# AnyLoc/Revisit-Anything

Measured on AMD Instinct MI355X. Metric: query_images_per_sec, higher is better.
Workload: dtype f32

## Files before the change

### revisit-anything_amd/csrc/api.hip

```cpp
#include <stdarg.h>
#include <stdlib.h>
#include <string.h>

#include <cmath>
#include <mutex>
#include <utility>

#include <initializer_list>

#include "ctx.h"

int segvlad_ctx::fail(int code, const char* fmt, ...) {
  va_list ap;
  va_start(ap, fmt);
  vsnprintf(err, sizeof(err), fmt, ap);
  va_end(ap);
  return code;
}

bool sv_is_device_ptr(const void* p) {
  hipPointerAttribute_t a;
  memset(&a, 0, sizeof(a));
  hipError_t e = hipPointerGetAttributes(&a, p);
  if (e != hipSuccess) {
// ... 199 lines not shown
  *out = c;
  return SEGVLAD_OK;
}

int segvlad_set_option(segvlad_ctx* ctx, const char* key, const char* value) {
  if (!ctx) return SEGVLAD_ERR_ARG;
  if (!key || !value) return ctx->fail(SEGVLAD_ERR_ARG, "set_option: null key/value");
  SvOptions& o = ctx->opt;
  auto as_int = [&](int* dst) -> int {
    char* end = nullptr;
    const long v = strtol(value, &end, 10);
    if (end == value || *end) return ctx->fail(SEGVLAD_ERR_ARG, "set_option(%s): '%s' is not an integer", key, value);
    *dst = (int)v;
    return SEGVLAD_OK;
  };
  if (!strcmp(key, "knn_filter")) {
    if (!strcmp(value, "auto")) o.knn_filter = 0;
    else if (!strcmp(value, "f16")) o.knn_filter = 1;
    else if (!strcmp(value, "bf16x3")) o.knn_filter = 2;
    else if (!strcmp(value, "fp32")) o.knn_filter = 3;
    else return ctx->fail(SEGVLAD_ERR_ARG, "set_option(knn_filter): want auto|f16|bf16x3|fp32, got '%s'", value);
    return SEGVLAD_OK;
  }
  if (!strcmp(key, "pca_arith")) {
    if (!strcmp(value, "auto") || !strcmp(value, "f16x3")) o.pca_fp32 = 0;
    else if (!strcmp(value, "fp32")) o.pca_fp32 = 1;
    else return ctx->fail(SEGVLAD_ERR_ARG, "set_option(pca_arith): want auto|f16x3|fp32, got '%s'", value);
    return SEGVLAD_OK;
  }
  if (!strcmp(key, "pca_path")) {
    if (!strcmp(value, "auto")) o.pca_path = 0;
    else if (!strcmp(value, "planes")) o.pca_path = 1;
    else if (!strcmp(value, "project")) o.pca_path = 2;
    else return ctx->fail(SEGVLAD_ERR_ARG, "set_option(pca_path): want auto|planes|project, got '%s'", value);
    return SEGVLAD_OK;
  }
  if (!strcmp(key, "vlad_assign")) {
    if (!strcmp(value, "hard")) {
      o.vlad_soft_temp = 0.f, o.vlad_soft_pooled = 0;
      return SEGVLAD_OK;
    }
    const int pooled = !strncmp(value, "soft_pooled:", 12);
    if (pooled || !strncmp(value, "soft:", 5)) {
      const char* t = value + (pooled ? 12 : 5);
      bool decimal = *t != 0 && (*t == '.' || (*t >= '0' && *t <= '9'));
      for (const char* c = t; *c && decimal; ++c) decimal = strchr("0123456789.eE+-", *c) != nullptr;
      char* end = nullptr;
      const float temp = decimal ? strtof(t, &end) : 0.f;
      if (decimal && end != t && *end == 0 && std::isfinite(temp) && temp > 0.f) {
        o.vlad_soft_temp = temp, o.vlad_soft_pooled = pooled;
        return SEGVLAD_OK;
      }
    }
    return ctx->fail(SEGVLAD_ERR_ARG, "set_option(vlad_assign): want hard|soft:<T>|soft_pooled:<T> with a finite decimal T > 0, got '%s'", value);
  }
  auto as_dev = [&](int* dst, std::initializer_list<int> product_values, std::initializer_list<int> probe_values = {}) -> int {
    int v = *dst;
    SV_TRY(as_int(&v));
    bool ok = false;
    for (int a : product_values) ok = ok || a == v;
#ifdef SEGVLAD_ABLATIONS
    for (int a : probe_values) ok = ok || a == v;
#else
    (void)probe_values;
#endif
    if (!ok)
      return ctx->fail(SEGVLAD_ERR_ARG, "set_option(%s=%d): a development switch -- this library holds the default kernels only "
                       "(SEGVLAD_BUILD_ABLATIONS=1 builds lib/libsegvlad_hip_abl.so with the probes of csrc/segvlad_dev.h)", key, v);
    *dst = v;
    return SEGVLAD_OK;
  };
  if (!strcmp(key, "f16_cfg")) return as_dev(&o.f16_cfg, {-1, 250, 300, 62, 63}, {93, 94, 95});
  if (!strcmp(key, "f16_gm")) return as_int(&o.f16_gm);
  if (!strcmp(key, "f16_walk")) return as_int(&o.f16_walk);
  if (!strcmp(key, "f16_deep_cfg")) return as_dev(&o.f16_deep_cfg, {-1, 4, 5});
  if (!strcmp(key, "f16_buf")) return as_dev(&o.f16_buf, {-1, 0});
  if (!strcmp(key, "tnk_gram")) return as_int(&o.tnk_gram);
  if (!strcmp(key, "tnk_fork")) return as_int(&o.tnk_fork);
  if (!strcmp(key, "x3_tile")) return as_int(&o.x3_tile);
  if (!strcmp(key, "x3_gm")) return as_int(&o.x3_gm);
  if (!strcmp(key, "search_stats")) return as_int(&o.search_stats);
  if (!strcmp(key, "knn_heuristic")) return as_int(&o.knn_heuristic);
  if (!strcmp(key, "assign_narrow")) return as_int(&o.assign_narrow);
  if (!strcmp(key, "agg_kpb")) return as_int(&o.agg_kpb);
  if (!strcmp(key, "pj_nw")) return as_int(&o.pj_nw);
  if (!strcmp(key, "pj_f16")) return as_int(&o.pj_f16);
  if (!strcmp(key, "cover_rows")) return as_int(&o.cover_rows);
  if (!strcmp(key, "pj_planes")) return as_int(&o.pj_planes);
  if (!strcmp(key, "small_plan")) return as_int(&o.small_plan);
  if (!strcmp(key, "small_tail")) return as_int(&o.small_tail);
  if (!strcmp(key, "small_head")) return as_int(&o.small_head);
  if (!strcmp(key, "batch_l0_f16")) return as_int(&o.batch_l0_f16);
  if (!strcmp(key, "level_carry")) return as_int(&o.level_carry);
  if (!strcmp(key, "f16_persist_wgs")) return as_int(&o.f16_persist_wgs);
  if (!strcmp(key, "debug_small_tail")) return as_int(&o.debug_small_tail);
  if (!strcmp(key, "refine_group")) return as_int(&o.refine_group);
  if (!strcmp(key, "query_group")) return as_int(&o.query_group);
  if (!strcmp(key, "group_fetch")) return as_int(&o.group_fetch);
  if (!strcmp(key, "debug_search")) return as_int(&o.debug_search);
  if (!strcmp(key, "debug_fail_search")) return as_int(&o.debug_fail_search);
  if (!strcmp(key, "guard_undersize")) {
    if (!ctx->guard) return ctx->fail(SEGVLAD_ERR_STATE, "set_option(guard_undersize): the context was not created under SEGVLAD_GUARD=1");
    const char* colon = strchr(value, ':');
    bool found = false;
    ctx->for_each_buf([&](DevBuf& b) {
      if (!colon) b.shrink = 0;
      else if (strlen(b.tag) == (size_t)(colon - value) && !strncmp(b.tag, value, (size_t)(colon - value))) {
        b.shrink = atoi(colon + 1);
        found = true;
      }
    });
    if (colon && !found) return ctx->fail(SEGVLAD_ERR_ARG, "set_option(guard_undersize): no buffer named like '%s'", value);
    return SEGVLAD_OK;
  }
  return ctx->fail(SEGVLAD_ERR_ARG, "set_option: unknown key '%s'", key);
}

int segvlad_destroy(segvlad_ctx* ctx) {
  if (!ctx) return SEGVLAD_OK;
  (void)hipSetDevice(ctx->device);
  (void)hipStreamSynchronize(ctx->stream);
  sv_comm_release(ctx);
  if (ctx->side) {
    (void)hipStreamSynchronize(ctx->side);
    (void)hipStreamDestroy(ctx->side);
    (void)hipEventDestroy(ctx->ev_fork);
    (void)hipEventDestroy(ctx->ev_join);
  }
  if (ctx->h_pin) {
    (void)hipHostFree(ctx->h_pin);
    (void)hipEventDestroy(ctx->ev_scalars);
  }
  if (ctx->h_desc) (void)hipHostFree(ctx->h_desc);
  if (ctx->ev_desc) (void)hipEventDestroy(ctx->ev_desc);
  ctx->for_each_buf([](DevBuf& b) { b.release(); });
  for (auto& kv : ctx->timers)
    for (hipEvent_t e : kv.second.ev)
      if (e) (void)hipEventDestroy(e);
  delete ctx;
  return SEGVLAD_OK;
}

const char* segvlad_last_error(const segvlad_ctx* ctx) { return ctx ? ctx->err : "null context"; }

int segvlad_set_stream(segvlad_ctx* ctx, void* hip_stream) {
  if (!ctx) return SEGVLAD_ERR_ARG;
  ctx->stream = reinterpret_cast<hipStream_t>(hip_stream);
  return SEGVLAD_OK;
}

int segvlad_synchronize(segvlad_ctx* ctx) {
  CHECK_CTX();
  SV_HIP(hipStreamSynchronize(ctx->stream));
  return sv_guard_check(ctx);
}

int segvlad_set_profiling(segvlad_ctx* ctx, int on) {
  if (!ctx) return SEGVLAD_ERR_ARG;
  ctx->profiling = on != 0;
  return SEGVLAD_OK;
}

int segvlad_profile_reset(segvlad_ctx* ctx) {
  if (!ctx) return SEGVLAD_ERR_ARG;
  for (auto& kv : ctx->timers) {
    kv.second.used = 0;
// ... 290 lines not shown
```

### revisit-anything_amd/csrc/ctx.h

```cpp
#pragma once
#include <hip/hip_runtime.h>
#include <math.h>
#include <stdint.h>
#include <stdio.h>
#include <string.h>

#include <map>
#include <string>
#include <vector>

#include "../../include/segvlad.h"

#define SV_HIP(expr)                                                                              \
  do {                                                                                            \
    hipError_t _e = (expr);                                                                       \
    if (_e != hipSuccess) {                                                                       \
      return ctx->fail(SEGVLAD_ERR_HIP, "%s failed: %s (%s:%d)", #expr, hipGetErrorString(_e),    \
                       __FILE__, __LINE__);                                                       \
    }                                                                                             \
  } while (0)

#define SV_TRY(expr)          \
  do {                        \
    int _r = (expr);          \
// ... 11 lines not shown
}
#endif

#if defined(__HIPCC__)
__host__ __device__
#endif
inline int sv_x3_swz(int64_t row) { return (int)((0 - (row >> 2)) & 3); }
#if defined(__HIPCC__)
__host__ __device__
#endif
inline size_t sv_x3_off(int64_t row, int64_t k, int64_t Kd) {
  return ((size_t)(row >> 7) * (size_t)(Kd >> 5) + (size_t)(k >> 5)) * 4096 + (size_t)(row & 127) * 32 +
         (size_t)((((k & 31) >> 3) ^ sv_x3_swz(row)) << 3) + (size_t)(k & 7);
}
inline int64_t sv_x3_rows(int64_t n) { return (n + 255) & ~255ll; }
inline float sv_fp16_scale(float bound) {
  int e;
  frexpf(bound, &e);
  return ldexpf(1.f, 14 - e);
}

constexpr size_t SV_GUARD_BYTES = 1024;
constexpr uint32_t SV_GUARD_WORD = 0xA5C3F00Du;
struct DevBuf {
  void* p = nullptr;
  size_t cap = 0;
  const char* tag = "";
  bool guard = false;
  bool fixed = false;
  void* raw = nullptr;
  size_t req = 0;
  int shrink = 0;
  hipError_t reserve(size_t bytes) {
    if (guard) return reserve_guarded(bytes);
    if (bytes <= cap) return hipSuccess;
    if (p) {
      hipError_t e = hipFree(p);
      if (e != hipSuccess) return e;
      p = nullptr;
      cap = 0;
    }
    size_t want = bytes + bytes / 8 + 256;
    hipError_t e = hipMalloc(&p, want);
    if (e != hipSuccess) return e;
    cap = want;
    return hipSuccess;
  }
  hipError_t reserve_guarded(size_t bytes);
  size_t fence_off() const { return fixed ? cap : ((req > (size_t)shrink ? req - (size_t)shrink : 0) + 3) & ~(size_t)3; }
  void release() {
    if (raw) (void)hipFree(raw);
    else if (p) (void)hipFree(p);
    raw = nullptr;
    p = nullptr;
    cap = 0;
    req = 0;
  }
  template <class T>
  T* as() { return reinterpret_cast<T*>(p); }
};

struct StageTimer {
  std::vector<hipEvent_t> ev;
  int used = 0;
  int launches = 0;
};

struct SvOptions {
  int knn_filter = 0;
  int pca_fp32 = 0;
  int f16_cfg = -1;
  int f16_gm = -1;
  int f16_walk = -1;
  int f16_persist_wgs = 32;
  int f16_deep_cfg = -1;
  int f16_buf = -1;
  int tnk_gram = 1;
  int tnk_fork = 1;
  int x3_tile = 0;
  int x3_gm = -1;
  int search_stats = 0;
  int knn_heuristic = 1;
  int assign_narrow = 0;
  int agg_kpb = 4;
  int debug_fail_search = 0;
  int debug_search = 0;
  int debug_small_tail = 0;
  int batch_l0_f16 = 1;
  int level_carry = 1;
  int small_head = 1;
  int small_tail = 1;
  int small_plan = 1;
  int pj_f16 = 1;
  int pj_nw = 8;
  int refine_group = 1;
  int query_group = 0;
  int pca_path = 0;
  int cover_rows = 1;
  int pj_planes = 1;
  float vlad_soft_temp = 0.f;
  int vlad_soft_pooled = 0;
  int group_fetch = 0;
};

constexpr int SV_F16_KBLOCK = 1024;
inline int sv_f16_kblock(const SvOptions& o, int d) {
  if (o.f16_cfg == 300) return SV_F16_KBLOCK;
  return (o.f16_cfg < 0 && d >= 4096) ? SV_F16_KBLOCK : 0;
}
constexpr int SV_F16_KFLUSH = 64;
int sv_f16_eps_kblock(const SvOptions& o, int d);
inline bool sv_f16_bias_possible(const SvOptions& o, int64_t nq) { return nq > 128 && (o.f16_cfg < 0 || o.f16_cfg == 250 || o.f16_cfg == 300); }
enum class F16Kernel {
  None, BatchDefault, BatchComplement, BatchSmall, BatchUnbiased, BatchUnbiasedSmall, DeepFlush, DeepFlushComplement, DeepBlockedBuf, DeepBlocked,
  DeepBlockedBufComplement, DeepBlockedComplement, DeepUnbiased, OneImage64, OneImage128,
#ifdef SEGVLAD_ABLATIONS
  ProbePhases, ProbeNoEpilogue, ProbeNoEpilogueNoDma,
#endif
};
struct F16Choice {
  F16Kernel kernel;
  const char* why;
};
F16Choice sv_choose_f16_kernel(const SvOptions& o, bool bias_ok, int M, int64_t n_rows, int d, int b_stride, int skip);
inline float sv_f16_c_eps(int d, int kb, float bias_mult) {
  const float acc = kb > 0 ? (2.f * (float)kb + (float)((d + kb - 1) / kb) + 1.f) / 16777216.f : 2.f * (float)d / 16777216.f;
  return 2.5f * (1.f / 1024.f + 1.f / 4194304.f + bias_mult * acc);
}

struct SvSearchStats {
  int64_t levels = 0;
  int64_t filter = 0;
  int64_t n_fallback = 0;
  int64_t cand_max = 0;
  int64_t cand_sum = 0;
  int64_t refine_max = 0;
  int64_t refine_sum = 0;
  int64_t n_queries = 0;
  int64_t n_redo = 0;
  int64_t n_refine2 = 0;
  int64_t grp_groups = 0;
  int64_t grp_union_sum = 0;
  int64_t carry_rows = 0;
};

struct OpenDescribe {
  bool open = false;
  bool side_pending = false;
  int B = 0, S_tot = 0;
  StageTimer* timer = nullptr;
  int slot = 0;
};

struct segvlad_ctx {
  int device = 0;
  hipStream_t stream = nullptr;
  hipStream_t side = nullptr;
  hipEvent_t ev_fork = nullptr, ev_join = nullptr;
  uint32_t* h_pin = nullptr;
  hipEvent_t ev_scalars = nullptr;
  unsigned char* h_desc = nullptr;
  size_t h_desc_cap = 0;
  hipEvent_t ev_desc = nullptr;
  OpenDescribe desc;
  char err[512] = {0};
  bool profiling = false;
// ... 318 lines not shown
```

### revisit-anything_amd/csrc/vlad_kernels.hip

```cpp
#include <stdio.h>
#include <stdlib.h>

#include "ctx.h"
#include "incidence_dev.h"

typedef float f32x16 __attribute__((ext_vector_type(16)));

#define MFMA32(a, b, c) __builtin_amdgcn_mfma_f32_32x32x2f32((a), (b), (c), 0, 0, 0)

template <int CTRL>
__device__ __forceinline__ float dpp_f32(float x) {
  return __int_as_float(__builtin_amdgcn_update_dpp(0, __float_as_int(x), CTRL, 0xf, 0xf, true));
}

__device__ __forceinline__ int frag_row(int r, int kk) { return (r & 3) + 8 * (r >> 2) + 4 * kk; }

__global__ void vocab_norm_kernel(const float* __restrict__ C, int K, int D, float* __restrict__ inv) {
  const int k = blockIdx.x;
  float s = 0.f;
  for (int d = threadIdx.x; d < D; d += blockDim.x) {
    float v = C[(size_t)k * D + d];
    s = fmaf(v, v, s);
  }
  __shared__ float red[256];
// ... 394 lines not shown
      const float* bp = bt + ((size_t)((dbase >> 1) + st) * NT) * 64 + l;
#pragma unroll
      for (int n = 0; n < NT; ++n) {
        const float bv = bp[n * 64];
        if (ABL == 1) {
          acc[0][n][0] += x0 * bv;
          acc[1][n][0] += x1 * bv;
        } else {
          acc[0][n] = MFMA32(x0, bv, acc[0][n]);
          acc[1][n] = MFMA32(x1, bv, acc[1][n]);
        }
      }
      if (ABL != 2) {
        tile[(2 * i) * 65 + 2 * st + kk] = x0;
        tile[(2 * i + 1) * 65 + 2 * st + kk] = x1;
      }
    }
    __builtin_amdgcn_fence(__ATOMIC_RELEASE, "wavefront");
    __builtin_amdgcn_wave_barrier();
    __builtin_amdgcn_fence(__ATOMIC_ACQUIRE, "wavefront");
#pragma unroll 4
    for (int it = 0; it < 16; ++it) {
      const int idx = it * 64 + l;
      const int tok = idx >> 4, c4 = (idx & 15) << 2;
      if (ABL != 2 && ABL != 3 && t0 + tok < N && dbase + c4 < D) {
        const float* q = tile + tok * 65 + c4;
        float4 v = make_float4(q[0], q[1], q[2], q[3]);
        *reinterpret_cast<float4*>(Xt + ((size_t)b * N + t0 + tok) * D + dbase + c4) = v;
      }
    }
    __builtin_amdgcn_fence(__ATOMIC_RELEASE, "wavefront");
    __builtin_amdgcn_wave_barrier();
    __builtin_amdgcn_fence(__ATOMIC_ACQUIRE, "wavefront");
  }
  ss0 += __shfl_xor(ss0, 32);
  ss1 += __shfl_xor(ss1, 32);
  __syncthreads();
  constexpr int KP = NT * 32;
  float* sc = lds;
  float* ssum = lds + 64 * (KP + 1);
  if (kk == 0) {
    ssum[w * 64 + 2 * i] = ss0;
    ssum[w * 64 + 2 * i + 1] = ss1;
  }
  for (int rnd = 0; rnd < 4; ++rnd) {
    if (w == rnd) {
#pragma unroll
      for (int mt = 0; mt < 2; ++mt)
#pragma unroll
        for (int n = 0; n < NT; ++n)
#pragma unroll
          for (int r = 0; r < 16; ++r) {
            const int tok = 2 * frag_row(r, kk) + mt;
            float* p = &sc[tok * (KP + 1) + n * 32 + i];
            *p = (rnd == 0) ? acc[mt][n][r] : (*p + acc[mt][n][r]);
          }
    }
    __syncthreads();
  }
  if (tid < 64 && t0 + tid < N) {
    const float s2 = ((ssum[tid] + ssum[64 + tid]) + ssum[128 + tid]) + ssum[192 + tid];
    const float rn = 1.0f / fmaxf(sqrtf(s2), 1e-12f);
    float best = -INFINITY, second = -INFINITY;
    int bi = 0;
    for (int k = 0; k < K; ++k) {
      const float v = sc[tid * (KP + 1) + k];
      if (v > best) {
        second = best;
        best = v;
        bi = k;
      } else if (v > second) {
        second = v;
      }
    }
    const size_t o = (size_t)b * N + t0 + tid;
    labels[o] = (uint8_t)bi;
    rnorm[o] = rn;
    if (gap) gap[o] = (K > 1) ? (best - second) * rn : INFINITY;
  }
}

typedef float f32x4u __attribute__((ext_vector_type(4), aligned(4)));

template <int NT>
__device__ __forceinline__ void assign_wide_chunk(const float* __restrict__ tl, const float* __restrict__ bt, float* __restrict__ Xt,
                                                  int b, int N, int D, int t0, int tid, int w, int l, int i, int kk, int c,
                                                  f32x16 (&acc)[NT], float& ss) {
  constexpr int DC = 32, TS = 128;
  auto rot = [](int d) { return 8 * (d >> 2) + 32 * (d & 1); };
#pragma unroll 8
  for (int st = 0; st < DC / 2; ++st) {
    const float x = tl[(2 * st + kk) * TS + ((32 * w + i + rot(2 * st + kk)) & 127)];
    ss = fmaf(x, x, ss);
    const float* bp = bt + ((size_t)(c * (DC / 2) + st) * NT) * 64 + l;
#pragma unroll
    for (int n = 0; n < NT; ++n) acc[n] = MFMA32(x, bp[n * 64], acc[n]);
  }
#pragma unroll
  for (int it = 0; it < 4; ++it) {
    const int idx = it * 256 + tid;
    const int tok = idx >> 3, c4 = idx & 7;
    if (t0 + tok < N) {
      const float* q = tl + (4 * c4) * TS;
      const int t_a = (tok + 8 * c4) & 127, t_b = (tok + 8 * c4 + 32) & 127;
      const float4 o = make_float4(q[t_a], q[TS + t_b], q[2 * TS + t_a], q[3 * TS + t_b]);
      *reinterpret_cast<float4*>(Xt + ((size_t)b * N + t0 + tok) * D + c * DC + 4 * c4) = o;
    }
  }
}

template <int NT>
__global__ __launch_bounds__(256) void assign_wide_kernel(const float* __restrict__ T, int N, int D, int K,
                                                          const float* __restrict__ bt, float* __restrict__ Xt,
                                                          uint8_t* __restrict__ labels, float* __restrict__ rnorm,
                                                          float* __restrict__ gap, int B) {
  constexpr int DC = 32, TS = 128;
  auto rot = [](int d) { return 8 * (d >> 2) + 32 * (d & 1); };
  __shared__ __attribute__((aligned(16))) float tile[2 * DC * TS + 128];
  __shared__ float ssum[128];
  const int gx = (N + 127) / 128;
  const int per = (int)((gridDim.x + 7) / 8);
  const int logical = (int)(blockIdx.x & 7) * per + (int)(blockIdx.x >> 3);
  if (logical >= gx * B) return;
  const int b = logical / gx, t0 = (logical - b * gx) * 128;
  const int tid = threadIdx.x, w = tid >> 6, l = tid & 63, i = l & 31, kk = l >> 5;
  const float* Tb = T + (size_t)b * D * N;
  const int lr = tid >> 5, lq = tid & 31;
  const int tl0 = t0 + 4 * lq;
  const int nvalid = N - tl0;
  f32x16 acc[NT];
#pragma unroll
  for (int n = 0; n < NT; ++n)
#pragma unroll
    for (int r = 0; r < 16; ++r) acc[n][r] = 0.f;
  float ss = 0.f;
  const int nch = D / DC;
  float4 va[4], vb[4];
#define SV_LOAD_CHUNK(V, c)                                                           \
  _Pragma("unroll") for (int j = 0; j < 4; ++j) {                                     \
    const float* p = Tb + (size_t)((c) * DC + lr + 8 * j) * N + tl0;                  \
    if (nvalid >= 4) {                                                                \
      const f32x4u u = *reinterpret_cast<const f32x4u*>(p);                           \
      V[j] = make_float4(u[0], u[1], u[2], u[3]);                                     \
    } else {                                                                          \
      V[j] = make_float4(nvalid > 0 ? p[0] : 0.f, nvalid > 1 ? p[1] : 0.f, nvalid > 2 ? p[2] : 0.f, 0.f); \
    }                                                                                 \
  }
#define SV_PARK_CHUNK(V, buf)                                                         \
  _Pragma("unroll") for (int j = 0; j < 4; ++j) {                                     \
    const int d_ = lr + 8 * j;                                                        \
    float* q = tile + (buf) * (DC * TS) + d_ * TS + ((4 * lq + rot(d_)) & 127);       \
    *reinterpret_cast<float4*>(q) = V[j];                                             \
  }
  SV_LOAD_CHUNK(va, 0)
  SV_PARK_CHUNK(va, 0)
  if (1 < nch) { SV_LOAD_CHUNK(va, 1) }
  __syncthreads();
#define SV_ASSIGN_STEP(c, VNEXT, VFREE)                                               \
  {                                                                                   \
    if ((c) + 2 < nch) { SV_LOAD_CHUNK(VFREE, (c) + 2) }                              \
    assign_wide_chunk<NT>(tile + ((c) & 1) * (DC * TS), bt, Xt, b, N, D, t0, tid, w, l, i, kk, (c), acc, ss);  \
    if ((c) + 1 < nch) { SV_PARK_CHUNK(VNEXT, ((c) + 1) & 1) }                        \
    __syncthreads();                                                                  \
  }
  for (int c = 0; c < nch; c += 2) {
    SV_ASSIGN_STEP(c, va, vb)
    if (c + 1 < nch) SV_ASSIGN_STEP(c + 1, vb, va)
  }
#undef SV_ASSIGN_STEP
#undef SV_LOAD_CHUNK
#undef SV_PARK_CHUNK
  constexpr int KP = NT * 32;
  float* sc = tile;
  ss += __shfl_xor(ss, 32);
  if (kk == 0) ssum[32 * w + i] = ss;
#pragma unroll
  for (int n = 0; n < NT; ++n)
#pragma unroll
    for (int r = 0; r < 16; ++r) sc[(32 * w + frag_row(r, kk)) * (KP + 1) + n * 32 + i] = acc[n][r];
  __syncthreads();
  if (tid < 128 && t0 + tid < N) {
    const float rn = 1.0f / fmaxf(sqrtf(ssum[tid]), 1e-12f);
    float best = -INFINITY, second = -INFINITY;
    int bi = 0;
    for (int k = 0; k < K; ++k) {
      const float sv = sc[tid * (KP + 1) + k];
      if (sv > best) {
        second = best;
        best = sv;
        bi = k;
      } else if (sv > second) {
        second = sv;
      }
    }
    const size_t o = (size_t)b * N + t0 + tid;
    labels[o] = (uint8_t)bi;
    rnorm[o] = rn;
    if (gap) gap[o] = (K > 1) ? (best - second) * rn : INFINITY;
  }
}

int sv_launch_assign(segvlad_ctx* ctx, const float* tokens, int B, int N, float* xt, uint8_t* labels, float* rnorm,
                     float* gap) {
  const int NT = ctx->Kpad / 32;
  dim3 grid((N + 63) / 64, B), block(256);
  const float* bt = ctx->vocab_bt.as<float>();
  if (NT <= 2 && ctx->D % 32 == 0 && !ctx->opt.assign_narrow) {
    const unsigned tiles_total = (unsigned)((N + 127) / 128) * (unsigned)B;
    dim3 gridw((tiles_total + 7) / 8 * 8, 1);
    if (NT == 1)
      hipLaunchKernelGGL(assign_wide_kernel<1>, gridw, block, 0, ctx->stream, tokens, N, ctx->D, ctx->K, bt, xt, labels, rnorm, gap, B);
    else
      hipLaunchKernelGGL(assign_wide_kernel<2>, gridw, block, 0, ctx->stream, tokens, N, ctx->D, ctx->K, bt, xt, labels, rnorm, gap, B);
    SV_HIP(hipGetLastError());
    return SEGVLAD_OK;
  }
  switch (NT) {
    case 1:
      hipLaunchKernelGGL(assign_kernel<1>, grid, block, 0, ctx->stream, tokens, N, ctx->D, ctx->K, bt, xt, labels, rnorm, gap);
      break;
    case 2: {
#ifdef SEGVLAD_ABLATIONS
      const char* ab = getenv("SEGVLAD_ASSIGN_ABL");
      const int a = ab ? atoi(ab) : 0;
      if (a == 1) {
        hipLaunchKernelGGL((assign_kernel<2, 1>), grid, block, 0, ctx->stream, tokens, N, ctx->D, ctx->K, bt, xt, labels, rnorm, gap);
        break;
      } else if (a == 2) {
        hipLaunchKernelGGL((assign_kernel<2, 2>), grid, block, 0, ctx->stream, tokens, N, ctx->D, ctx->K, bt, xt, labels, rnorm, gap);
        break;
      } else if (a == 3) {
        hipLaunchKernelGGL((assign_kernel<2, 3>), grid, block, 0, ctx->stream, tokens, N, ctx->D, ctx->K, bt, xt, labels, rnorm, gap);
        break;
      }
#endif
      hipLaunchKernelGGL(assign_kernel<2>, grid, block, 0, ctx->stream, tokens, N, ctx->D, ctx->K, bt, xt, labels, rnorm, gap);
      break;
    }
    case 4:
      hipLaunchKernelGGL(assign_kernel<4>, grid, block, 0, ctx->stream, tokens, N, ctx->D, ctx->K, bt, xt, labels, rnorm, gap);
      break;
    default:
      return ctx->fail(SEGVLAD_ERR_LIMIT, "K=%d: supported cluster counts are 1..64 and 97..128 (Kpad in {32,64,128})", ctx->K);
  }
  SV_HIP(hipGetLastError());
  return SEGVLAD_OK;
}

__global__ __launch_bounds__(256) void prep_kernel(const uint8_t* __restrict__ labels, const uint64_t* __restrict__ inc,
                                                   const int32_t* __restrict__ seg_off,
                                                   const int64_t* __restrict__ adj_off, const uint8_t* __restrict__ adj,
                                                   int N, int K, int S_max, int SC, uint64_t* __restrict__ colmask,
                                                   float* __restrict__ gscale, int32_t* __restrict__ tok_order,
                                                   int32_t* __restrict__ lab_off, const float* __restrict__ rnorm,
                                                   float* __restrict__ rn_sorted, int stage, int ord_n,
                                                   int32_t* __restrict__ phys, int32_t* __restrict__ cov_cnt, int cover) {
  extern __shared__ __attribute__((aligned(16))) unsigned char smem[];
  const int b = blockIdx.x;
  const int nw = (N + 63) >> 6;
  const int s0 = seg_off[b], S = seg_off[b + 1] - s0;
  uint64_t* inc2 = reinterpret_cast<uint64_t*>(smem);
  uint64_t* lbits = inc2 + (size_t)S_max * nw;
  const int tid = threadIdx.x;
  if (adj && stage) {
    const int SW = (S_max + 63) >> 6;
    uint64_t* inc0 = reinterpret_cast<uint64_t*>(reinterpret_cast<int*>(lbits + (size_t)K * nw) + ord_n);
    uint64_t* nbr = inc0 + (size_t)S_max * nw;
    for (int idx = tid; idx < S * nw; idx += 256) inc0[idx] = inc[(size_t)s0 * nw + idx];
    for (int idx = tid; idx < S * SW; idx += 256) nbr[idx] = 0;
    __syncthreads();
    const uint8_t* a = adj + adj_off[b];
    for (int e = tid; e < S * S; e += 256)
      if (a[e]) {
        const int s = e / S, u = e - s * S;
        atomicOr(reinterpret_cast<unsigned long long*>(&nbr[s * SW + (u >> 6)]), 1ull << (u & 63));
      }
    __syncthreads();
    for (int idx = tid; idx < S * nw; idx += 256) {
      const int s = idx / nw, w = idx - s * nw;
      uint64_t v = 0;
      for (int uw = 0; uw < SW; ++uw) {
        uint64_t m = nbr[s * SW + uw];
        while (m) {
          const int u = (uw << 6) + __builtin_ctzll(m);
          m &= m - 1;
          v |= inc0[u * nw + w];
        }
      }
      inc2[idx] = v;
    }
  } else {
    for (int idx = tid; idx < S * nw; idx += 256) {
// ... 453 lines not shown
        if (single && dummy_row >= 0) {
          if (f >= TNK_QD && rem >= TNK_QD - 1) {
            if (sc == 0) asm volatile("s_waitcnt vmcnt(23)" ::: "memory");
            else asm volatile("s_waitcnt vmcnt(7)" ::: "memory");
          } else {
            tnk_wait_vm((rem < TNK_QD - 1 ? rem : TNK_QD - 1) + (sc == 0 ? 2 * (f < TNK_QD ? f : TNK_QD) : 0));
          }
        } else {
          asm volatile("s_waitcnt vmcnt(0)" ::: "memory");
        }
        if (single)
          lds_step_read(lds_addr(qbase + (f % TNK_QD) * 1024 + l * 16), lds_addr(rnl + j), lds_addr(mskl + j), x, rn, m);
        else
          x = lds_read_f32x4(lds_addr(qbase + (f % TNK_QD) * 1024 + l * 16));
        if (fi < total) issue();
        if (!dvalid) x = f32x4{0.f, 0.f, 0.f, 0.f};
        const float b0 = fmaf(x.x, rn, -c4.x), b1 = fmaf(x.y, rn, -c4.y);
        const float b2 = fmaf(x.z, rn, -c4.z), b3 = fmaf(x.w, rn, -c4.w);
        if (sc == 0) {
          typedef _Float16 h4 __attribute__((ext_vector_type(4)));
          const float fv[4] = {b0 * xscale, b1 * xscale, b2 * xscale, b3 * xscale};
          h4 p1, p2;
#pragma unroll
          for (int e = 0; e < 4; ++e) {
            p1[e] = (_Float16)fv[e];
            p2[e] = (_Float16)(fv[e] - (float)p1[e]);
          }
          if (single) prw = lds_read_i32(lds_addr(rowl + j));
          const bool real = dvalid && prw >= 0;
          const unsigned rr = (unsigned)prw;
          const size_t ob = real ? ((size_t)(rr >> 7) * nkb_d + kb_dc) * 4096 + (size_t)(((rr & 127u) << 5) + (((lane_c ^ (unsigned)sv_x3_swz(rr)) << 3) | lane_o))
                                 : ob_dummy;
          *reinterpret_cast<h4*>(h1 + ob) = p1;
          *reinterpret_cast<h4*>(h2 + ob) = p2;
        }
        const float a0 = ((m >> i) & 1ull) ? 1.f : 0.f;
        acc[0][0] = MFMA32(a0, b0, acc[0][0]);
        acc[0][1] = MFMA32(a0, b1, acc[0][1]);
        acc[0][2] = MFMA32(a0, b2, acc[0][2]);
        acc[0][3] = MFMA32(a0, b3, acc[0][3]);
        if (two) {
          const float a1 = ((m >> (32 + i)) & 1ull) ? 1.f : 0.f;
          acc[1][0] = MFMA32(a1, b0, acc[1][0]);
          acc[1][1] = MFMA32(a1, b1, acc[1][1]);
          acc[1][2] = MFMA32(a1, b2, acc[1][2]);
          acc[1][3] = MFMA32(a1, b3, acc[1][3]);
        }
      }
#pragma unroll
      for (int mt = 0; mt < 2; ++mt) {
        if (mt == 1 && !two) break;
#pragma unroll
        for (int r = 0; r < 16; ++r) {
          float q2 = nsq[mt][r];
#pragma unroll
          for (int q = 0; q < 4; ++q) {
            q2 = fmaf(acc[mt][q][r], acc[mt][q][r], q2);
            acc[mt][q][r] = 0.f;
          }
          nsq[mt][r] = q2;
        }
      }
    }
#pragma unroll
    for (int mt = 0; mt < 2; ++mt) {
      if (mt == 1 && !two) break;
#pragma unroll
      for (int r = 0; r < 16; ++r) {
        float p = nsq[mt][r];
        p += dpp_f32<0xB1>(p);
        p += dpp_f32<0x4E>(p);
        p += dpp_f32<0x141>(p);
        p += dpp_f32<0x140>(p);
        p += __shfl_xor(p, 16);
        const int row = 32 * mt + frag_row(r, kk);
        if (i == 0 && row < Sc) block_norms[(size_t)(s0 + 64 * sc + row) * K + k] = sqrtf(p);
      }
    }
  }
}

constexpr int GNK_SLOT = 4096;

template <int T, int QS>
__global__ __launch_bounds__(T == 1 ? 256 : 128, 2) void gram_norms_kernel(const float* __restrict__ Xt, const float* __restrict__ rnorm,
                                                                         const int32_t* __restrict__ tok_order,
                                                                         const int32_t* __restrict__ lab_off,
                                                                         const uint64_t* __restrict__ colmask,
                                                                         const float* __restrict__ C,
                                                                         const int32_t* __restrict__ seg_off, int N, int D, int K, int SC,
                                                                         float* __restrict__ block_norms, float xscale,
                                                                         _Float16* __restrict__ h1, _Float16* __restrict__ h2,
                                                                         const int32_t* __restrict__ rowbase, int safe_waits,
                                                                         uint8_t* __restrict__ redo_task,
                                                                         const int32_t* __restrict__ phys, int64_t dummy_row) {
  extern __shared__ __attribute__((aligned(16))) unsigned char smem[];
  typedef _Float16 f16x8 __attribute__((ext_vector_type(8)));
  constexpr int WAVES = T == 1 ? 4 : 2;
  constexpr int NG = T * (T + 1) / 2;
  const int b = blockIdx.y;
  const int tid = threadIdx.x, l = tid & 63, i = l & 31, kk = l >> 5;
  const int w = __builtin_amdgcn_readfirstlane(tid >> 6);
  const int k = (int)blockIdx.x * WAVES + w;
  if (k >= K) return;
  const size_t wsz = (size_t)QS * T * GNK_SLOT + (size_t)D * 4;
  unsigned char* qbase = smem + (size_t)w * wsz;
  float* cl = reinterpret_cast<float*>(qbase + QS * T * GNK_SLOT);
  const int o0 = lab_off[(size_t)b * (K + 1) + k];
  const int n = lab_off[(size_t)b * (K + 1) + k + 1] - o0;
  if (n > 32 * T || (T == 2 && n <= 32)) return;
  const int s0 = seg_off[b], S = seg_off[b + 1] - s0;
  if (n == 0) {
    for (int s = l; s < S; s += 64) block_norms[(size_t)(s0 + s) * K + k] = 0.f;
    return;
  }
  const size_t tb = (size_t)b * N + o0;
  for (int d = 4 * l; d < D; d += 256) *reinterpret_cast<float4*>(cl + d) = *reinterpret_cast<const float4*>(C + (size_t)k * D + d);
  bool real[T];
  float rn[T];
#pragma unroll
  for (int tt = 0; tt < T; ++tt) {
    real[tt] = 32 * tt + i < n;
    rn[tt] = real[tt] ? rnorm[tb + 32 * tt + i] : 0.f;
  }
  const float* Xb = Xt + (size_t)b * N * D;
  const float* src[4 * T];
#pragma unroll
  for (int pz = 0; pz < 4 * T; ++pz) {
    const int jj = 8 * pz + (l >> 3);
    const int t = jj < n ? tok_order[tb + jj] : tok_order[tb];
    src[pz] = Xb + (size_t)t * D + 4 * ((l & 7) ^ ((jj >> 1) & 7));
  }
  const int steps = D >> 5;
  const int NP = (n + 7) >> 3;
  auto issue = [&](int f) {
#pragma unroll
    for (int pz = 0; pz < 4 * T; ++pz)
      if (pz < NP) {
        if (8 * pz + (l >> 3) < n)
          __builtin_amdgcn_global_load_lds((agg_gptr_t)(src[pz] + 32 * f), (agg_lptr_t)(qbase + (f % QS) * (T * GNK_SLOT) + pz * 1024), 16, 0, 0);
      }
  };
#pragma unroll
  for (int q = 0; q < QS; ++q)
    if (q < steps) issue(q);
  f32x16 acc[NG];
#pragma unroll
  for (int g = 0; g < NG; ++g)
#pragma unroll
    for (int r = 0; r < 16; ++r) acc[g][r] = 0.f;
  size_t prow[T];
  unsigned pswz[T];
#pragma unroll
  for (int tt = 0; tt < T; ++tt) {
    const int ph = real[tt] ? phys[tb + 32 * tt + i] : 0;
    const int64_t rr = ph >= 0 ? (int64_t)rowbase[(size_t)b * K + k] + ph : dummy_row + ((32 * (k + tt) + i) & 255);
    prow[tt] = (size_t)(rr >> 7) * (size_t)(D >> 5) * 4096 + (size_t)(rr & 127) * 32;
    pswz[tt] = (unsigned)sv_x3_swz(rr);
  }
  const unsigned fsw = (unsigned)((i >> 1) & 7);
  const unsigned a_tok = lds_addr(qbase) + (unsigned)i * 128u;
  for (int f = 0; f < steps; ++f) {
    if (f >= QS && f + QS - 1 < steps && !safe_waits) tnk_wait_vm(QS * 4 * T + (QS - 1) * NP);
    else asm volatile("s_waitcnt vmcnt(0)" ::: "memory");
    f32x4 x[T][4], c[4];
    {
      const unsigned ac = lds_addr(cl) + (unsigned)(32 * f + 8 * kk) * 4u;
      const unsigned p0 = ((unsigned)(2 * kk) ^ fsw) << 4, p1 = ((unsigned)(2 * kk + 1) ^ fsw) << 4;
      const unsigned p2 = ((unsigned)(4 + 2 * kk) ^ fsw) << 4, p3 = ((unsigned)(5 + 2 * kk) ^ fsw) << 4;
#pragma unroll
      for (int tt = 0; tt < T; ++tt) {
        const unsigned a0 = a_tok + (unsigned)(f % QS) * (T * GNK_SLOT) + (unsigned)tt * GNK_SLOT;
        asm volatile("ds_read_b128 %0, %4\n\tds_read_b128 %1, %5\n\tds_read_b128 %2, %6\n\tds_read_b128 %3, %7"
                     : "=&v"(x[tt][0]), "=&v"(x[tt][1]), "=&v"(x[tt][2]), "=&v"(x[tt][3])
                     : "v"(a0 + p0), "v"(a0 + p1), "v"(a0 + p2), "v"(a0 + p3)
                     : "memory");
      }
      asm volatile("ds_read_b128 %0, %4\n\tds_read_b128 %1, %4 offset:16\n\tds_read_b128 %2, %4 offset:64\n\tds_read_b128 %3, %4 offset:80\n\t"
                   "s_waitcnt lgkmcnt(0)"
                   : "=&v"(c[0]), "=&v"(c[1]), "=&v"(c[2]), "=&v"(c[3])
                   : "v"(ac)
                   : "memory");
#pragma unroll
      for (int tt = 0; tt < T; ++tt) asm volatile("" : "+v"(x[tt][0]), "+v"(x[tt][1]), "+v"(x[tt][2]), "+v"(x[tt][3]));
    }
    if (f + QS < steps) issue(f + QS);
    asm volatile("" ::: "memory");
#pragma unroll
    for (int ks = 0; ks < 2; ++ks) {
      f16x8 hh[T], ll[T];
#pragma unroll
      for (int tt = 0; tt < T; ++tt) {
#pragma unroll
        for (int e = 0; e < 8; ++e) {
          const float xv = x[tt][2 * ks + (e >> 2)][e & 3], cv = c[2 * ks + (e >> 2)][e & 3];
          const float fv = real[tt] ? fmaf(xv, rn[tt], -cv) * xscale : 0.f;
          hh[tt][e] = (_Float16)fv;
          ll[tt][e] = (_Float16)(fv - (float)hh[tt][e]);
        }
        const size_t ob = prow[tt] + (size_t)f * 4096 + (size_t)((((unsigned)(2 * ks + kk)) ^ pswz[tt]) << 3);
        if (real[tt]) {
          *reinterpret_cast<f16x8*>(h1 + ob) = hh[tt];
          *reinterpret_cast<f16x8*>(h2 + ob) = ll[tt];
        }
      }
#pragma unroll
      for (int ta = 0, g = 0; ta < T; ++ta)
#pragma unroll
        for (int tb2 = ta; tb2 < T; ++tb2, ++g) {
          acc[g] = __builtin_amdgcn_mfma_f32_32x32x16_f16(ll[ta], hh[tb2], acc[g], 0, 0, 0);
          acc[g] = __builtin_amdgcn_mfma_f32_32x32x16_f16(hh[ta], ll[tb2], acc[g], 0, 0, 0);
          acc[g] = __builtin_amdgcn_mfma_f32_32x32x16_f16(hh[ta], hh[tb2], acc[g], 0, 0, 0);
        }
    }
  }
  float dgl[T];
#pragma unroll
  for (int tt = 0; tt < T; ++tt) {
    dgl[tt] = 0.f;
    const int gd = tt == 0 ? 0 : NG - 1;
#pragma unroll
    for (int r = 0; r < 16; ++r)
      if (frag_row(r, kk) == i) dgl[tt] = acc[gd][r];
  }
  bool cancels = false;
  const float inv_x2 = 1.f / (xscale * xscale);
  const int SCb = (S + 63) >> 6;
  for (int sc = 0; sc < SCb; ++sc) {
    const int Sc = min(64, S - 64 * sc);
    uint64_t mt[T];
#pragma unroll
    for (int tt = 0; tt < T; ++tt) mt[tt] = real[tt] ? colmask[(tb + 32 * tt + i) * SC + sc] : 0ull;
    for (int s = 0; s < Sc; ++s) {
      uint32_t W[T];
      bool any = false;
#pragma unroll
      for (int tt = 0; tt < T; ++tt) {
        W[tt] = (uint32_t)__builtin_amdgcn_ballot_w64(((mt[tt] >> s) & 1ull) != 0ull);
        any |= W[tt] != 0u;
      }
      float p = 0.f;
      if (any) {
#pragma unroll
        for (int ta = 0, g = 0; ta < T; ++ta)
#pragma unroll
          for (int tb2 = ta; tb2 < T; ++tb2, ++g) {
            float q = 0.f;
#pragma unroll
            for (int r = 0; r < 16; ++r) q += ((W[ta] >> frag_row(r, kk)) & 1u) ? acc[g][r] : 0.f;
            q = ((W[tb2] >> i) & 1u) ? q : 0.f;
            p += (ta == tb2) ? q : 2.f * q;
          }
        p += dpp_f32<0xB1>(p);
        p += dpp_f32<0x4E>(p);
        p += dpp_f32<0x141>(p);
        p += dpp_f32<0x140>(p);
        p += __shfl_xor(p, 16);
        p += __shfl_xor(p, 32);
        float dg = 0.f;
#pragma unroll
        for (int tt = 0; tt < T; ++tt) dg += ((W[tt] >> i) & 1u) ? dgl[tt] : 0.f;
        dg += dpp_f32<0xB1>(dg);
        dg += dpp_f32<0x4E>(dg);
        dg += dpp_f32<0x141>(dg);
        dg += dpp_f32<0x140>(dg);
        dg += __shfl_xor(dg, 16);
        dg += __shfl_xor(dg, 32);
        cancels = cancels || (p < 0.0625f * dg);
      }
      if (l == 0) block_norms[(size_t)(s0 + 64 * sc + s) * K + k] = sqrtf(fmaxf(p, 0.f) * inv_x2);
    }
  }
  if (cancels && l == 0 && redo_task) redo_task[(size_t)b * K + k] = 1;
}

int sv_launch_token_norms(segvlad_ctx* ctx, const float* xt, const uint64_t* colmask, const float* centres, int K, int D,
                          const int32_t* seg_off_dev, int B, int N, int SC, float* block_norms, float xscale, uint16_t* h1,
                          uint16_t* h2, const int32_t* rowbase, int64_t dummy_row, const int32_t* phys) {
  if (D % 4) return ctx->fail(SEGVLAD_ERR_ARG, "token_norms: D=%d must be a multiple of 4", D);
  const int Dpad = (D + 127) & ~127;
  const size_t lds = (size_t)TNK_WAVES * ((size_t)TNK_QD * 1024 + (size_t)TNK_LCAP * 20 + (size_t)Dpad * 4);
  if (lds > 160 * 1024) return ctx->fail(SEGVLAD_ERR_LIMIT, "token_norms: D=%d needs %zu B of LDS", D, lds);
  const bool gram = ctx->opt.tnk_gram != 0 && (D % 32) == 0;
  const int skip_le = gram ? 64 : -1;
  uint8_t* redo_task = nullptr;
  if (gram) {
    SV_HIP(ctx->s_tnk_redo.reserve((size_t)B * K));
    redo_task = ctx->s_tnk_redo.as<uint8_t>();
    SV_HIP(hipMemsetAsync(redo_task, 0, (size_t)B * K, ctx->stream));
    const bool fork = N > 32 && ctx->opt.tnk_fork != 0;
    if (fork) SV_TRY(sv_fork_side(ctx));
    for (int T = 2; T >= 1; --T) {
      if (T == 2 && N <= 32) continue;
      const int waves = T == 1 ? 4 : 2;
      const int qs = T == 1 ? 3 : 2;
      const size_t glds = (size_t)waves * ((size_t)qs * T * GNK_SLOT + (size_t)D * 4);
      auto gk = T == 1 ? gram_norms_kernel<1, 3> : gram_norms_kernel<2, 2>;
      if (glds > 64 * 1024) SV_HIP(sv_max_dyn_lds(reinterpret_cast<const void*>(gk), glds));
      hipLaunchKernelGGL(gk, dim3((K + waves - 1) / waves, B), dim3(64 * waves), glds, (T == 2 && fork) ? ctx->side : ctx->stream, xt,
                         ctx->s_rnsorted.as<float>(), ctx->s_tokorder.as<int32_t>(), ctx->s_laboff.as<int32_t>(), colmask, centres,
                         seg_off_dev, N, D, K, SC, block_norms, xscale, reinterpret_cast<_Float16*>(h1),
                         reinterpret_cast<_Float16*>(h2), rowbase, dummy_row < 0 ? 1 : 0, redo_task, phys,
                         dummy_row < 0 ? -dummy_row : dummy_row);
      SV_HIP(hipGetLastError());
    }
    if (fork) SV_TRY(sv_join_side(ctx));
  }
  for (int big = 0; big < 2; ++big) {
    if (big && N < TNK_LCAP) break;
    auto kern = big ? token_norms_kernel<true> : token_norms_kernel<false>;
    if (lds > 64 * 1024)
      SV_HIP(sv_max_dyn_lds(reinterpret_cast<const void*>(kern), (size_t)lds));
    hipLaunchKernelGGL(kern, dim3((K + TNK_WAVES - 1) / TNK_WAVES, B), dim3(64 * TNK_WAVES), lds, ctx->stream, xt,
                       ctx->s_rnsorted.as<float>(), ctx->s_tokorder.as<int32_t>(), ctx->s_laboff.as<int32_t>(), colmask, centres,
                       seg_off_dev, N, D, K, SC, Dpad, block_norms, xscale, reinterpret_cast<_Float16*>(h1),
                       reinterpret_cast<_Float16*>(h2), rowbase, dummy_row, skip_le, redo_task, phys);
    SV_HIP(hipGetLastError());
  }
  return SEGVLAD_OK;
}

int sv_launch_aggregate(segvlad_ctx* ctx, const float* xt, const float* ,
                        const uint8_t* ,
                        const uint64_t* colmask, const float* centres, int K, int D, const int32_t* seg_off_dev,
                        const float* gscale, int B, int N, int SC, float* out, float* block_norms, const float* mean,
                        float xscale, uint16_t* h1, uint16_t* h2) {
  const int nwaves = (D + 127) / 128;
  if (nwaves > 12)
    return ctx->fail(SEGVLAD_ERR_LIMIT, "aggregate: D=%d exceeds the 1536-wide workgroup of this build", D);
  const int Ncap = (N + 2) & ~1;
  const int PW = nwaves * 2 + 1;
  size_t lds = (size_t)Ncap * 16 + (size_t)(64 * PW + 64) * sizeof(float) + 16 * sizeof(int);
  lds = (lds + 15) & ~(size_t)15;
  lds += (size_t)nwaves * 6 * 1024;
  if (lds > 160 * 1024) return ctx->fail(SEGVLAD_ERR_LIMIT, "aggregate: N=%d tokens need %zu B of LDS (limit 160 KiB)", N, lds);
  auto kern = (h1 != nullptr) ? aggregate_kernel<true> : aggregate_kernel<false>;
  bool phases = false;
#ifdef SEGVLAD_ABLATIONS
  if (const char* ab = getenv("SEGVLAD_AGG_ABL")) {
    if (atoi(ab) == 1) kern = aggregate_kernel<false, 1>;
    if (atoi(ab) == 2) kern = aggregate_kernel<false, 2>;
    if (atoi(ab) == 9) {
      kern = aggregate_kernel<false, 9>;
      phases = true;
      unsigned long long z[8] = {0, 0, 0, 0, 0, 0, 0, 0};
      SV_HIP(hipMemcpyToSymbol(HIP_SYMBOL(sv_agg_phase_cycles), z, sizeof(z)));
    }
  }
#endif
  if (lds > 64 * 1024)
    SV_HIP(sv_max_dyn_lds(reinterpret_cast<const void*>(kern), (size_t)lds));
  int kpb = ctx->opt.agg_kpb;
  if (kpb < 1) kpb = 1;
  hipLaunchKernelGGL(kern, dim3((K + kpb - 1) / kpb, B), dim3(nwaves * 64), lds, ctx->stream, xt, ctx->s_rnsorted.as<float>(),
                     ctx->s_tokorder.as<int32_t>(),
                     ctx->s_laboff.as<int32_t>(), colmask, centres, seg_off_dev,
                     gscale, N, D, K, SC, Ncap, out, block_norms, mean, xscale, reinterpret_cast<_Float16*>(h1),
                     reinterpret_cast<_Float16*>(h2), kpb);
  SV_HIP(hipGetLastError());
#ifdef SEGVLAD_ABLATIONS
  if (phases) {
    unsigned long long c8[8];
    SV_HIP(hipStreamSynchronize(ctx->stream));
    SV_HIP(hipMemcpyFromSymbol(c8, HIP_SYMBOL(sv_agg_phase_cycles), sizeof(c8)));
    double tot = 0;
    for (int q = 0; q < 8; ++q) tot += (double)c8[q];
    fprintf(stderr, "[aggregate phases] lists %.1f%% main %.1f%% | partial norms %.1f%% barrier %.1f%% row sums %.1f%% barrier %.1f%% | stores %.1f%% barrier %.1f%% (%.0f cycles per (k, image))\n",
            100 * c8[0] / tot, 100 * c8[1] / tot, 100 * c8[5] / tot, 100 * c8[6] / tot, 100 * c8[7] / tot, 100 * c8[2] / tot,
            100 * c8[3] / tot, 100 * c8[4] / tot, tot / ((double)K * B));
  }
#endif
  (void)phases;
  return SEGVLAD_OK;
}
```

Baseline: 8787.

## Share centre row across batch waves in T=1 gram_norms and deepen load queue

For the T=1 gram_norms kernel the default now maps one centre per block across several batch images (one wave each). The centre vector is staged once in shared LDS instead of per wave, and the freed LDS funds a 4-deep load queue instead of 3, with a wider vmcnt wait helper. Ablation variants of the assign and gram kernels are added behind a build flag and do not run by default. The new grid shape changes block count and occupancy and adds a block-wide sync before the per-wave work.

```diff
diff --git a/revisit-anything_amd/csrc/api.hip b/revisit-anything_amd/csrc/api.hip
--- a/revisit-anything_amd/csrc/api.hip
+++ b/revisit-anything_amd/csrc/api.hip
@@ -305,6 +305,9 @@
   if (!strcmp(key, "search_stats")) return as_int(&o.search_stats);
   if (!strcmp(key, "knn_heuristic")) return as_int(&o.knn_heuristic);
   if (!strcmp(key, "assign_narrow")) return as_int(&o.assign_narrow);
+  if (!strcmp(key, "gram_queue")) return as_dev(&o.gram_queue, {3, 4}, {5, 6});
+  if (!strcmp(key, "assign_abl")) return as_dev(&o.assign_abl, {0}, {1, 2, 3});
+  if (!strcmp(key, "gram_abl")) return as_dev(&o.gram_abl, {0}, {1, 2, 3, 4});
   if (!strcmp(key, "agg_kpb")) return as_int(&o.agg_kpb);
   if (!strcmp(key, "pj_nw")) return as_int(&o.pj_nw);
   if (!strcmp(key, "pj_f16")) return as_int(&o.pj_f16);
diff --git a/revisit-anything_amd/csrc/ctx.h b/revisit-anything_amd/csrc/ctx.h
--- a/revisit-anything_amd/csrc/ctx.h
+++ b/revisit-anything_amd/csrc/ctx.h
@@ -117,6 +117,9 @@
   int search_stats = 0;
   int knn_heuristic = 1;
   int assign_narrow = 0;
+  int gram_queue = 4;
+  int assign_abl = 0;
+  int gram_abl = 0;
   int agg_kpb = 4;
   int debug_fail_search = 0;
   int debug_search = 0;
diff --git a/revisit-anything_amd/csrc/vlad_kernels.hip b/revisit-anything_amd/csrc/vlad_kernels.hip
--- a/revisit-anything_amd/csrc/vlad_kernels.hip
+++ b/revisit-anything_amd/csrc/vlad_kernels.hip
@@ -500,7 +500,7 @@
 
 typedef float f32x4u __attribute__((ext_vector_type(4), aligned(4)));
 
-template <int NT>
+template <int NT, int ABL>
 __device__ __forceinline__ void assign_wide_chunk(const float* __restrict__ tl, const float* __restrict__ bt, float* __restrict__ Xt,
                                                   int b, int N, int D, int t0, int tid, int w, int l, int i, int kk, int c,
                                                   f32x16 (&acc)[NT], float& ss) {
@@ -510,10 +510,12 @@
   for (int st = 0; st < DC / 2; ++st) {
     const float x = tl[(2 * st + kk) * TS + ((32 * w + i + rot(2 * st + kk)) & 127)];
     ss = fmaf(x, x, ss);
+    if (ABL == 2) continue;
     const float* bp = bt + ((size_t)(c * (DC / 2) + st) * NT) * 64 + l;
 #pragma unroll
     for (int n = 0; n < NT; ++n) acc[n] = MFMA32(x, bp[n * 64], acc[n]);
   }
+  if (ABL == 1) return;
 #pragma unroll
   for (int it = 0; it < 4; ++it) {
     const int idx = it * 256 + tid;
@@ -527,7 +529,7 @@
   }
 }
 
-template <int NT>
+template <int NT, int ABL = 0>
 __global__ __launch_bounds__(256) void assign_wide_kernel(const float* __restrict__ T, int N, int D, int K,
                                                           const float* __restrict__ bt, float* __restrict__ Xt,
                                                           uint8_t* __restrict__ labels, float* __restrict__ rnorm,
@@ -570,6 +572,26 @@
     float* q = tile + (buf) * (DC * TS) + d_ * TS + ((4 * lq + rot(d_)) & 127);       \
     *reinterpret_cast<float4*>(q) = V[j];                                             \
   }
+  if (ABL == 3) {
+#define SV_EAT_CHUNK(V) _Pragma("unroll") for (int j = 0; j < 4; ++j) ss += (V[j].x + V[j].y) + (V[j].z + V[j].w);
+    SV_LOAD_CHUNK(va, 0)
+    if (1 < nch) { SV_LOAD_CHUNK(vb, 1) }
+    for (int c = 0; c < nch; c += 2) {
+      SV_EAT_CHUNK(va)
+      if (c + 2 < nch) { SV_LOAD_CHUNK(va, c + 2) }
+      if (c + 1 < nch) {
+        SV_EAT_CHUNK(vb)
+        if (c + 3 < nch) { SV_LOAD_CHUNK(vb, c + 3) }
+      }
+    }
+#undef SV_EAT_CHUNK
+    if (tid < 128 && t0 + tid < N) {
+      labels[(size_t)b * N + t0 + tid] = (uint8_t)((t0 + tid) % K);
+      rnorm[(size_t)b * N + t0 + tid] = ss == 12345.678f ? ss : 1.f;
+      if (gap) gap[(size_t)b * N + t0 + tid] = 1.f;
+    }
+    return;
+  }
   SV_LOAD_CHUNK(va, 0)
   SV_PARK_CHUNK(va, 0)
   if (1 < nch) { SV_LOAD_CHUNK(va, 1) }
@@ -577,7 +599,7 @@
 #define SV_ASSIGN_STEP(c, VNEXT, VFREE)                                               \
   {                                                                                   \
     if ((c) + 2 < nch) { SV_LOAD_CHUNK(VFREE, (c) + 2) }                              \
-    assign_wide_chunk<NT>(tile + ((c) & 1) * (DC * TS), bt, Xt, b, N, D, t0, tid, w, l, i, kk, (c), acc, ss);  \
+    assign_wide_chunk<NT, ABL>(tile + ((c) & 1) * (DC * TS), bt, Xt, b, N, D, t0, tid, w, l, i, kk, (c), acc, ss);  \
     if ((c) + 1 < nch) { SV_PARK_CHUNK(VNEXT, ((c) + 1) & 1) }                        \
     __syncthreads();                                                                  \
   }
@@ -626,6 +648,14 @@
   if (NT <= 2 && ctx->D % 32 == 0 && !ctx->opt.assign_narrow) {
     const unsigned tiles_total = (unsigned)((N + 127) / 128) * (unsigned)B;
     dim3 gridw((tiles_total + 7) / 8 * 8, 1);
+#ifdef SEGVLAD_ABLATIONS
+    if (NT == 2 && ctx->opt.assign_abl) {
+      auto ak = ctx->opt.assign_abl == 1 ? assign_wide_kernel<2, 1> : ctx->opt.assign_abl == 2 ? assign_wide_kernel<2, 2> : assign_wide_kernel<2, 3>;
+      hipLaunchKernelGGL(ak, gridw, block, 0, ctx->stream, tokens, N, ctx->D, ctx->K, bt, xt, labels, rnorm, gap, B);
+      SV_HIP(hipGetLastError());
+      return SEGVLAD_OK;
+    }
+#endif
     if (NT == 1)
       hipLaunchKernelGGL(assign_wide_kernel<1>, gridw, block, 0, ctx->stream, tokens, N, ctx->D, ctx->K, bt, xt, labels, rnorm, gap, B);
     else
@@ -1245,8 +1275,19 @@
 
 constexpr int GNK_SLOT = 4096;
 
-template <int T, int QS>
-__global__ __launch_bounds__(T == 1 ? 256 : 128, 2) void gram_norms_kernel(const float* __restrict__ Xt, const float* __restrict__ rnorm,
+__device__ __forceinline__ void gnk_wait_vm(int n) {
+#define GNK_W(v) case v: asm volatile("s_waitcnt vmcnt(" #v ")" ::: "memory"); break;
+  switch (n) {
+    GNK_W(0) GNK_W(1) GNK_W(2) GNK_W(3) GNK_W(4) GNK_W(5) GNK_W(6) GNK_W(7) GNK_W(8) GNK_W(9) GNK_W(10) GNK_W(11) GNK_W(12) GNK_W(13)
+    GNK_W(14) GNK_W(15) GNK_W(16) GNK_W(17) GNK_W(18) GNK_W(19) GNK_W(20) GNK_W(21) GNK_W(22) GNK_W(23) GNK_W(24) GNK_W(25) GNK_W(26)
+    GNK_W(27) GNK_W(28) GNK_W(29) GNK_W(30) GNK_W(31) GNK_W(32) GNK_W(33) GNK_W(34) GNK_W(35) GNK_W(36) GNK_W(37) GNK_W(38) GNK_W(39)
+    default: asm volatile("s_waitcnt vmcnt(40)" ::: "memory"); break;
+  }
+#undef GNK_W
+}
+
+template <int T, int QS, bool SHC = false, int WV = (T == 1 ? 4 : 2), int ABL = 0>
+__global__ __launch_bounds__(64 * WV, 2) void gram_norms_kernel(const float* __restrict__ Xt, const float* __restrict__ rnorm,
                                                                          const int32_t* __restrict__ tok_order,
                                                                          const int32_t* __restrict__ lab_off,
                                                                          const uint64_t* __restrict__ colmask,
@@ -1256,19 +1297,26 @@
                                                                          _Float16* __restrict__ h1, _Float16* __restrict__ h2,
                                                                          const int32_t* __restrict__ rowbase, int safe_waits,
                                                                          uint8_t* __restrict__ redo_task,
-                                                                         const int32_t* __restrict__ phys, int64_t dummy_row) {
+                                                                         const int32_t* __restrict__ phys, int64_t dummy_row, int B) {
   extern __shared__ __attribute__((aligned(16))) unsigned char smem[];
   typedef _Float16 f16x8 __attribute__((ext_vector_type(8)));
-  constexpr int WAVES = T == 1 ? 4 : 2;
+  constexpr int WAVES = WV;
   constexpr int NG = T * (T + 1) / 2;
-  const int b = blockIdx.y;
+  constexpr int NST = (ABL == 1 || ABL == 3) ? 0 : 4 * T;
   const int tid = threadIdx.x, l = tid & 63, i = l & 31, kk = l >> 5;
   const int w = __builtin_amdgcn_readfirstlane(tid >> 6);
-  const int k = (int)blockIdx.x * WAVES + w;
-  if (k >= K) return;
-  const size_t wsz = (size_t)QS * T * GNK_SLOT + (size_t)D * 4;
+  const int b = SHC ? (int)blockIdx.y * WAVES + w : (int)blockIdx.y;
+  const int k = SHC ? (int)blockIdx.x : (int)blockIdx.x * WAVES + w;
+  const size_t wsz = (size_t)QS * T * GNK_SLOT + (SHC ? (size_t)0 : (size_t)D * 4);
   unsigned char* qbase = smem + (size_t)w * wsz;
-  float* cl = reinterpret_cast<float*>(qbase + QS * T * GNK_SLOT);
+  float* cl = reinterpret_cast<float*>(SHC ? smem + (size_t)WAVES * wsz : qbase + QS * T * GNK_SLOT);
+  if (SHC) {
+    for (int d = 4 * tid; d < D; d += 256 * WAVES) *reinterpret_cast<float4*>(cl + d) = *reinterpret_cast<const float4*>(C + (size_t)k * D + d);
+    __syncthreads();
+    if (b >= B) return;
+  } else {
+    if (k >= K) return;
+  }
   const int o0 = lab_off[(size_t)b * (K + 1) + k];
   const int n = lab_off[(size_t)b * (K + 1) + k + 1] - o0;
   if (n > 32 * T || (T == 2 && n <= 32)) return;
@@ -1278,7 +1326,8 @@
     return;
   }
   const size_t tb = (size_t)b * N + o0;
-  for (int d = 4 * l; d < D; d += 256) *reinterpret_cast<float4*>(cl + d) = *reinterpret_cast<const float4*>(C + (size_t)k * D + d);
+  if (!SHC)
+    for (int d = 4 * l; d < D; d += 256) *reinterpret_cast<float4*>(cl + d) = *reinterpret_cast<const float4*>(C + (size_t)k * D + d);
   bool real[T];
   float rn[T];
 #pragma unroll
@@ -1324,9 +1373,17 @@
   const unsigned fsw = (unsigned)((i >> 1) & 7);
   const unsigned a_tok = lds_addr(qbase) + (unsigned)i * 128u;
   for (int f = 0; f < steps; ++f) {
-    if (f >= QS && f + QS - 1 < steps && !safe_waits) tnk_wait_vm(QS * 4 * T + (QS - 1) * NP);
-    else asm volatile("s_waitcnt vmcnt(0)" ::: "memory");
+    if (f >= QS && f + QS - 1 < steps && !safe_waits) {
+      if (SHC) gnk_wait_vm(QS * NST + (QS - 1) * NP);
+      else tnk_wait_vm(QS * NST + (QS - 1) * NP);
+    } else {
+      asm volatile("s_waitcnt vmcnt(0)" ::: "memory");
+    }
     f32x4 x[T][4], c[4];
+    if (ABL == 3) {
+      if (f + QS < steps) issue(f + QS);
+      continue;
+    }
     {
       const unsigned ac = lds_addr(cl) + (unsigned)(32 * f + 8 * kk) * 4u;
       const unsigned p0 = ((unsigned)(2 * kk) ^ fsw) << 4, p1 = ((unsigned)(2 * kk + 1) ^ fsw) << 4;
@@ -1362,7 +1419,10 @@
           ll[tt][e] = (_Float16)(fv - (float)hh[tt][e]);
         }
         const size_t ob = prow[tt] + (size_t)f * 4096 + (size_t)((((unsigned)(2 * ks + kk)) ^ pswz[tt]) << 3);
-        if (real[tt]) {
+        if (ABL == 4 && real[tt]) {
+          __builtin_nontemporal_store(hh[tt], reinterpret_cast<f16x8*>(h1 + ob));
+          __builtin_nontemporal_store(ll[tt], reinterpret_cast<f16x8*>(h2 + ob));
+        } else if (ABL != 1 && real[tt]) {
           *reinterpret_cast<f16x8*>(h1 + ob) = hh[tt];
           *reinterpret_cast<f16x8*>(h2 + ob) = ll[tt];
         }
@@ -1371,6 +1431,10 @@
       for (int ta = 0, g = 0; ta < T; ++ta)
 #pragma unroll
         for (int tb2 = ta; tb2 < T; ++tb2, ++g) {
+          if (ABL == 2) {
+            acc[g][0] += (float)ll[ta][0] + (float)hh[tb2][7];
+            continue;
+          }
           acc[g] = __builtin_amdgcn_mfma_f32_32x32x16_f16(ll[ta], hh[tb2], acc[g], 0, 0, 0);
           acc[g] = __builtin_amdgcn_mfma_f32_32x32x16_f16(hh[ta], ll[tb2], acc[g], 0, 0, 0);
           acc[g] = __builtin_amdgcn_mfma_f32_32x32x16_f16(hh[ta], hh[tb2], acc[g], 0, 0, 0);
@@ -1455,16 +1519,36 @@
     if (fork) SV_TRY(sv_fork_side(ctx));
     for (int T = 2; T >= 1; --T) {
       if (T == 2 && N <= 32) continue;
-      const int waves = T == 1 ? 4 : 2;
-      const int qs = T == 1 ? 3 : 2;
-      const size_t glds = (size_t)waves * ((size_t)qs * T * GNK_SLOT + (size_t)D * 4);
-      auto gk = T == 1 ? gram_norms_kernel<1, 3> : gram_norms_kernel<2, 2>;
+      typedef decltype(&gram_norms_kernel<1, 3>) gram_kernel_t;
+      gram_kernel_t gk = gram_norms_kernel<2, 2>;
+      int waves = 2, qs = 2;
+      bool shc = false;
+      if (T == 1) {
+        const int gq = ctx->opt.gram_queue;
+        gk = gq == 3 ? gram_norms_kernel<1, 3> : gram_norms_kernel<1, 4, true>;
+        waves = 4, qs = gq == 3 ? 3 : 4, shc = gq != 3;
+#ifdef SEGVLAD_ABLATIONS
+        if (gq == 5) gk = gram_norms_kernel<1, 3, true, 6>, waves = 6, qs = 3;
+        if (gq == 6) gk = gram_norms_kernel<1, 5, true, 3>, waves = 3, qs = 5;
+        const int a = ctx->opt.gram_abl;
+        if (gq == 3 && a == 1) gk = gram_norms_kernel<1, 3, false, 4, 1>;
+        if (gq == 3 && a == 2) gk = gram_norms_kernel<1, 3, false, 4, 2>;
+        if (gq == 3 && a == 3) gk = gram_norms_kernel<1, 3, false, 4, 3>;
+        if (gq == 4 && a == 1) gk = gram_norms_kernel<1, 4, true, 4, 1>;
+        if (gq == 4 && a == 2) gk = gram_norms_kernel<1, 4, true, 4, 2>;
+        if (gq == 4 && a == 3) gk = gram_norms_kernel<1, 4, true, 4, 3>;
+        if (gq == 4 && a == 4) gk = gram_norms_kernel<1, 4, true, 4, 4>;
+#endif
+      }
+      const size_t glds = shc ? (size_t)waves * qs * T * GNK_SLOT + (size_t)D * 4 : (size_t)waves * ((size_t)qs * T * GNK_SLOT + (size_t)D * 4);
+      if (glds > 160 * 1024) return ctx->fail(SEGVLAD_ERR_LIMIT, "gram_norms: D=%d needs %zu B of LDS", D, glds);
       if (glds > 64 * 1024) SV_HIP(sv_max_dyn_lds(reinterpret_cast<const void*>(gk), glds));
-      hipLaunchKernelGGL(gk, dim3((K + waves - 1) / waves, B), dim3(64 * waves), glds, (T == 2 && fork) ? ctx->side : ctx->stream, xt,
+      const dim3 ggrid = shc ? dim3(K, (B + waves - 1) / waves) : dim3((K + waves - 1) / waves, B);
+      hipLaunchKernelGGL(gk, ggrid, dim3(64 * waves), glds, (T == 2 && fork) ? ctx->side : ctx->stream, xt,
                          ctx->s_rnsorted.as<float>(), ctx->s_tokorder.as<int32_t>(), ctx->s_laboff.as<int32_t>(), colmask, centres,
                          seg_off_dev, N, D, K, SC, block_norms, xscale, reinterpret_cast<_Float16*>(h1),
                          reinterpret_cast<_Float16*>(h2), rowbase, dummy_row < 0 ? 1 : 0, redo_task, phys,
-                         dummy_row < 0 ? -dummy_row : dummy_row);
+                         dummy_row < 0 ? -dummy_row : dummy_row, B);
       SV_HIP(hipGetLastError());
     }
     if (fork) SV_TRY(sv_join_side(ctx));
```

After: 8779. No clear change (-0.1%).
